# bdsaglam/torch-scae

Hardware: AMD Instinct MI355X
Metric: images/sec SCAE fwd+bwd, MNIST 40x40 bs=128, 1/2/4/8 MI355X (higher is better)
Workload: dtype f32

## Files before the change

include/scae_hip.h:

```cpp
#ifndef SCAE_HIP_H
#define SCAE_HIP_H

#include <stdint.h>

#ifdef __cplusplus
extern "C" {
#endif

#define SCAE_ABI_VERSION 3

#define SCAE_OK 0
#define SCAE_ERR_BAD_ARG (-1)
#define SCAE_ERR_UNSUPPORTED (-2)

#define SCAE_MAX_CHANNELS 4
#define SCAE_ATTN_MAX_SET 64
#define SCAE_RENDER_MAX_TEMPLATE_ELEMS 4096

int scae_abi_version(void);
const char *scae_error_string(int code);

void *scae_launch_list_begin(void *stream);
int scae_launch_list_end(void *list);
int scae_launch_list_size(const void *list);
// ... 188 lines not shown
  const float *all_param;
  const float *cpr_static, *bias_cvr, *bias_caps, *bias_vote, *bias_scale;
  const float *noise_caps, *noise_vote;
  float noise_scale;
  int V, ld_param, similarity, learn_vote_scale, allow_deformations;
  float *vote, *scale, *vote_presence, *logit_caps, *logit_vote, *reg_partial;
  float *caps_presence;
  int *caps_arg;
  const float *gvote, *gscale, *gvote_presence, *glogit_caps, *glogit_vote, *greg;
  const float *gcaps_presence;
  float *gall_param, *gcpr_in, *gall_param_gated;
} scae_votes_desc;
int scae_mlp_chain_votes_fwd_f32(const scae_mlp_chain_desc *desc, const scae_votes_desc *votes,
                                 void *stream);
int scae_mlp_chain_votes_bwd_f32(const scae_mlp_chain_desc *desc, const scae_votes_desc *votes,
                                 void *stream);

int scae_gemm_bf16(const float *A, const float *B, float *C, const float *bias,
                   const float *mask, float *asum, int batch, int M, int N, int K,
                   int a_kcontig, int lda, int64_t a_batch, int b_kcontig, int ldb,
                   int64_t b_batch, int ldc, int64_t c_batch, int bias_ld, int64_t bias_batch,
                   int ldmask, int64_t mask_batch, int64_t asum_batch, int asum_ld, int relu,
                   void *stream);
int scae_gemm_pair_bf16(const scae_gemm_desc *first, const scae_gemm_desc *second, void *stream);
int scae_gemm_multi_bf16(const scae_gemm_desc *descs, int n, void *stream);
int scae_conv3x3_fwd_fold_f32(const float *in, const float *wf, const float *bias, float *out,
                              const float *post_bias, float *out_post, int B, int IH, int IW,
                              int Cin, int Cout, int stride, const scae_seed_fold_desc *fold,
                              void *stream);
int scae_conv3x3_fwd_res_supported(int B, int IH, int IW, int Cin, int Cout, int stride);
int scae_conv3x3_fwd_res_f32(const float *in, const float *wp, const float *bias, float *out,
                             const float *post_bias, float *out_post, int B, int IH, int IW,
                             int Cin, int Cout, int stride, int group, void *stream);
int scae_conv3x3_fwd_bf16(const float *in, const float *wf, const float *bias, float *out,
                          const float *post_bias, float *out_post, int B, int IH, int IW, int Cin,
                          int Cout, int stride, void *stream);
int scae_conv3x3_bwd_pair_bf16(const float *dpre, const float *wd, const float *in, float *din,
                               float *partial, int B, int IH, int IW, int Cin, int Cout,
                               int stride, void *stream);

int64_t scae_conv3x3_wf_floats(int Cout, int Cin);
int scae_conv3x3_relayout_f32(const float *w, float *wf, float *wd, int Cout, int Cin,
                              void *stream);

int scae_conv3x3_bf16r_supported(int B, int IH, int IW, int Cin, int Cout, int stride);
int scae_conv3x3_first_fwd_relayout_bf16(const float *img, const float *w, const float *bias,
                                         uint16_t *out_h, int B, int Cin, int IH, int IW,
                                         int Cout, int stride, int n_layers,
                                         const float *const *rw, float *const *rwf,
                                         float *const *rwd, uint16_t *const *rwfh,
                                         uint16_t *const *rwdh, const int *rCout,
                                         const int *rCin, void *stream);
int scae_cvt_bf16_batch(int n_arrays, const float *const *src, uint16_t *const *dst,
                        const int64_t *n, void *stream);
int scae_conv3x3_fwd_bf16r(const uint16_t *in, const uint16_t *wf, const float *bias,
                           uint16_t *out_h, float *out_f, const float *post_bias,
                           float *out_post, int B, int IH, int IW, int Cin, int Cout, int stride,
                           void *stream);
int scae_conv3x3_dgrad_bf16r(const uint16_t *dpre, const uint16_t *wd, const uint16_t *gate,
                             uint16_t *din_h, float *din_f, int B, int IH, int IW, int Cin,
                             int Cout, int stride, void *stream);
int scae_conv3x3_wgrad_bf16r_splits(int B, int OH, int OW, int Cin, int Cout);
int scae_conv3x3_wgrad_bf16r(const uint16_t *dpre, const uint16_t *x, float *partial, int B,
                             int IH, int IW, int Cin, int Cout, int stride, void *stream);
int scae_conv3x3_relayout_batch_f32(int n_layers, const float *const *w, float *const *wf,
                                    float *const *wd, const int *Cout, const int *Cin,
// ... 555 lines not shown
```

torch_scae_amd/_lib.py:

```python
import ctypes
import os
from ctypes import (POINTER, Structure, c_char_p, c_double, c_float, c_int,
                    c_int64, c_uint32, c_uint64, c_void_p)

_HERE = os.path.dirname(os.path.abspath(__file__))
LIB_PATH = os.environ.get("SCAE_HIP_LIB") or os.path.join(_HERE, "lib",
                                                        "libscae_hip.so")

P = c_void_p


class DecoderDesc(Structure):
    _fields_ = [("templates", P), ("templates_alpha", P), ("pose", P),
                ("presence", P), ("bg_image", P), ("bg_value", P),
                ("bg_mixing_logit", P), ("temperature_logit", P),
                ("out_scale", P),
                ("B", c_int), ("M", c_int), ("C", c_int), ("th", c_int),
                ("tw", c_int), ("H", c_int), ("W", c_int),
                ("template_repeat", c_int)]


class LikelihoodBwdDesc(Structure):
    _fields_ = [(n, P) for n in (
        "vote", "scale", "vote_presence", "dummy_vote", "x", "presence",
# ... 174 lines not shown
    "scae_gemm_pair_f32": [POINTER(GemmDesc), POINTER(GemmDesc), P],
    "scae_launch_list_begin": [P],
    "scae_launch_list_end": [P],
    "scae_launch_list_size": [P],
    "scae_launch_list_run": [P, P],
    "scae_launch_list_lane": [P, c_int],
    "scae_launch_list_timeline": [P, P, P, POINTER(c_float), c_int],
    "scae_launch_list_free": [P],
    "scae_gemm_multi_f32": [POINTER(GemmDesc), c_int, P],
    "scae_gemm_multi_bf16": [POINTER(GemmDesc), c_int, P],
    "scae_mlp_chain_max_width": [],
    "scae_mlp_chain_fwd_f32": [POINTER(MlpChainDesc), P],
    "scae_mlp_chain_bwd_f32": [POINTER(MlpChainDesc), P],
    "scae_mlp_chain_votes_fwd_f32": [POINTER(MlpChainDesc), POINTER(VotesDesc), P],
    "scae_mlp_chain_votes_bwd_f32": [POINTER(MlpChainDesc), POINTER(VotesDesc), P],
    "scae_gemm_pair_bf16": [POINTER(GemmDesc), POINTER(GemmDesc), P],
    "scae_conv3x3_wf_floats": [c_int, c_int],
    "scae_conv3x3_relayout_f32": [P, P, P, c_int, c_int, P],
    "scae_conv3x3_bf16r_supported": [c_int] * 6,
    "scae_conv3x3_first_fwd_relayout_bf16": [P] * 4 + [c_int] * 7 + [P] * 8,
    "scae_cvt_bf16_batch": [c_int, P, P, P, P],
    "scae_conv3x3_fwd_bf16r": [P] * 7 + [c_int] * 6 + [P],
    "scae_conv3x3_dgrad_bf16r": [P] * 5 + [c_int] * 6 + [P],
    "scae_conv3x3_wgrad_bf16r_splits": [c_int] * 5,
    "scae_conv3x3_wgrad_bf16r": [P] * 3 + [c_int] * 6 + [P],
    "scae_conv3x3_relayout_batch_f32": [c_int, P, P, P, P, P, P],
    "scae_conv3x3_first_fwd_f32": [P] * 4 + [c_int] * 6 + [P],
    "scae_conv3x3_first_fwd_relayout_f32": [P] * 4 + [c_int] * 7 + [P] * 6,
    "scae_conv3x3_first_wgrad_reduce_f32": [P] * 3 + [c_int] * 7 + [P] * 7,
    "scae_conv3x3_first_wgrad_rows": [c_int] * 2,
    "scae_conv3x3_first_wgrad_f32": [P] * 3 + [c_int] * 6 + [P],
    "scae_conv3x3_fwd_f32": [P] * 6 + [c_int] * 6 + [P],
    "scae_conv3x3_fwd_fold_f32": [P] * 6 + [c_int] * 6 + [POINTER(SeedFoldDesc), P],
    "scae_conv3x3_fwd_res_supported": [c_int] * 6,
    "scae_conv3x3_fwd_res_f32": [P] * 6 + [c_int] * 7 + [P],
    "scae_conv3x3_fwd_bf16": [P] * 6 + [c_int] * 6 + [P],
    "scae_conv3x3_dgrad_f32": [P] * 4 + [c_int] * 6 + [P],
    "scae_conv3x3_bwd_pair_f32": [P] * 5 + [c_int] * 6 + [P],
    "scae_conv3x3_bwd_pair_reduce_f32": [P] * 5 + [c_int] * 6 + [P, c_int] + [P] * 7
    + [c_int] * 2 + [P],
    "scae_conv3x3_bwd_pair_fold_f32": [P] * 5 + [c_int] * 6
    + [POINTER(SeedFoldDesc), POINTER(SeedFoldGrads), P],
    "scae_conv3x3_bwd_pair_bf16": [P] * 5 + [c_int] * 6 + [P],
    "scae_conv3x3_wgrad_reduce_batch_f32": [c_int] + [P] * 7,
    "scae_conv3x3_wgrad_splits": [c_int] * 5,
    "scae_conv3x3_wgrad_f32": [P] * 5 + [c_int] * 6 + [P],
    "scae_attention_pool_supported": [c_int] * 3,
    "scae_attention_pool_fwd_f32": [P, P] + [c_int] * 4 + [P],
    "scae_attention_pool_bwd_f32": [P, P, P] + [c_int] * 4 + [P],
    "scae_stage_batch": [P, P, c_int64, P, P, c_int64, P],
    "scae_step_prologue_f32": [P, P, c_int64, P, P, c_int64, P, c_int64, P,
                               POINTER(SeedFoldDesc), P],
    "scae_step_prologue_first_f32": [P, P, c_int64, P, P, c_int64, P, c_int64,
                                     P, POINTER(SeedFoldDesc),
                                     POINTER(FirstLayerDesc), P],
    "scae_gather_batch_f32": [P, P, c_int, POINTER(BatchSourceDesc), P],
    "scae_step_prologue_source_f32": [P, P, c_int, POINTER(BatchSourceDesc), P, c_int64, P,
                                      POINTER(SeedFoldDesc), POINTER(FirstLayerDesc), P],
    "scae_rmsprop_step_f32": [P, P, P, P, c_int64, c_float, P, c_float, c_float,
                              c_float, c_float, c_float, P],
    "scae_rmsprop_sums_step_f32": [P, P, P, P, c_int64, c_float, P, c_float, c_float,
                                   c_float, c_float, POINTER(SumJob), c_int, P],
    "scae_flat_opt_step_f32": [P, P, P, P, P, c_int64, P, P, c_int, c_double, c_double, c_float,
                               c_float, c_float, c_int, c_float, c_int, P],
    "scae_flat_opt_sums_step_f32": [P, P, P, P, P, c_int64, P, P, c_int, c_double, c_double,
                                    c_float, c_float, c_int, c_float, POINTER(SumJob), c_int, P],
# ... 204 lines not shown
```

torch_scae_amd/csrc/conv_mfma.hip:

```cpp
#include <cstdlib>

#include "mfma_tile.h"
#include "mfma_pipe.h"
#include "conv_first_dev.h"
#include "seed_fold_dev.h"

#include <algorithm>

#include "wave_mfma.h"

#define SCAE_DEVICE_ONLY
namespace scae_sf {
#include "seed_fold.hip"
}
namespace scae_saw {
#include "seed_attention_wave.hip"
}
#undef SCAE_DEVICE_ONLY

namespace {
using namespace scae_tile;

using scae_first::ConvGeom;

// ... 801 lines not shown
      for (int j = 0; j < 4; ++j)
        pipe::dma16(ra, reinterpret_cast<float *>(stage + 8 * j * ROWB), va[j], sa);
    } else {
#pragma unroll
      for (int j = 0; j < 4; ++j) {
        const int row = 8 * j + (lane >> 3);
        const int dh = pih[j] - kh, dw = piw[j] - kw, oh = dh >> 1, ow = dw >> 1;
        const bool ok = pn[j] >= 0 && dh >= 0 && dw >= 0 && oh < g.OH && ow < g.OW;
        const int vv = ok ? ((pn[j] + oh * g.OW + ow) * g.Cout) * 4 + swz(row, lane & 7) * 16
                          : pipe::DMA_ZERO;
        pipe::dma16(ra, reinterpret_cast<float *>(stage + 8 * j * ROWB), vv, h * BKF * 4);
      }
    }
#pragma unroll
    for (int j = 0; j < 8; ++j)
      pipe::dma16(rb, reinterpret_cast<float *>(stage + A_B + 8 * j * ROWB), vb[j], sb);
  });
  const int row = tid >> 3, c8 = 8 * (tid & 7), m = m0 + row;
  if (m >= M) return;
  const int nb = m / (AH * AW), rem = m - nb * AH * AW, a = rem / AW, b = rem - a * AW;
  const int ih = pl.rlist[pl.rstart[rc] + a], iw = pl.clist[pl.cstart[cc] + b];
  const size_t o = (((size_t)nb * g.IH + ih) * g.IW + iw) * g.Cin + n0 + c8;
  if (gate) {
    const float4 g0 = ld4(gate + o), g1 = ld4(gate + o + 4);
    v.lo.x = g0.x > 0.f ? v.lo.x : 0.f, v.lo.y = g0.y > 0.f ? v.lo.y : 0.f;
    v.lo.z = g0.z > 0.f ? v.lo.z : 0.f, v.lo.w = g0.w > 0.f ? v.lo.w : 0.f;
    v.hi.x = g1.x > 0.f ? v.hi.x : 0.f, v.hi.y = g1.y > 0.f ? v.hi.y : 0.f;
    v.hi.z = g1.z > 0.f ? v.hi.z : 0.f, v.hi.w = g1.w > 0.f ? v.hi.w : 0.f;
  }
  *reinterpret_cast<float4 *>(din + o) = v.lo;
  *reinterpret_cast<float4 *>(din + o + 4) = v.hi;
}

template <int DMODE>
struct DgradShape {
  static constexpr int SMEM = Tile<DMODE>::SMEM;
};
template <>
struct DgradShape<4> {
  static constexpr int SMEM = dgx::SMEM;
};
template <>
struct DgradShape<5> {
  static constexpr int SMEM = dgk::SMEM;
};
template <int DMODE, int SM>
__device__ __forceinline__ void dgrad_any_tile(float *smem, int bx, int by,
                                               const float *__restrict__ dpre,
                                               const float *__restrict__ wd,
                                               const float *__restrict__ gate,
                                               float *__restrict__ din, const ConvGeom &g,
                                               const DgradPlan &pl) {
  if constexpr (DMODE == 4)
    dgrad_x6_tile<(SM >= 2 * dgx::SMEM ? 2 : 1)>(smem, bx, by, dpre, wd, gate, din, g, pl);
  else if constexpr (DMODE == 5)
    dgrad_x6k_tile(smem, bx, by, dpre, wd, gate, din, g, pl);
  else
    dgrad_tile<DMODE>(smem, bx, by, dpre, wd, gate, din, g, pl);
}

template <int NS>
__global__ __launch_bounds__(NT) void conv_dgrad_x6_kernel(const float *__restrict__ dpre,
                                                           const float *__restrict__ wd,
                                                           const float *__restrict__ gate,
                                                           float *__restrict__ din, ConvGeom g,
                                                           DgradPlan pl) {
// ... 399 lines not shown
  if (lds > 64 * 1024) return SCAE_ERR_UNSUPPORTED;
  ReduceBatch r{};
  int rb = 0;
  if (n_layers > 0) {
    rb = fill_reduce(r, n_layers, rpartial, rdw, rdb, rCout, rCin, rsplits);
    SCAE_REQUIRE(rb > 0);
  }
  const int n_first = B * f.slices;
#define SCAE_FIRST_WGRAD(CI)                                                                  \
  case CI:                                                                                    \
    scae::launch(conv_first_wgrad_kernel<CI>, dim3(n_first + n_layers * rb), dim3(256), \
                       lds, (hipStream_t)stream, dpre, img, partial, g, r, n_first, rb);      \
    break;
  switch (Cin) {
    SCAE_FIRST_WGRAD(1) SCAE_FIRST_WGRAD(2) SCAE_FIRST_WGRAD(3) SCAE_FIRST_WGRAD(4)
    default: return SCAE_ERR_UNSUPPORTED;
  }
#undef SCAE_FIRST_WGRAD
  return scae_launch_status();
}

extern "C" int scae_conv3x3_first_wgrad_f32(const float *dpre, const float *img, float *partial,
                                            int B, int Cin, int IH, int IW, int Cout, int stride,
                                            void *stream) {
  return scae_conv3x3_first_wgrad_reduce_f32(dpre, img, partial, B, Cin, IH, IW, Cout, stride, 0,
                                             nullptr, nullptr, nullptr, nullptr, nullptr, nullptr,
                                             stream);
}

static bool conv_bf16_shape(long rows, int Cin, int Cout) {
  return Cin % 128 == 0 && Cout % 128 == 0 && rows * (Cout / 128) >= 128 * 128;
}

static int conv_fwd_impl(const float *in, const float *wf, const float *bias, float *out,
                         const float *post_bias, float *out_post, int B, int IH, int IW, int Cin,
                         int Cout, int stride, bool bf16, void *stream) {
  ConvGeom g{B, IH, IW, (IH - 3) / stride + 1, (IW - 3) / stride + 1, Cin, Cout, stride};
  int rc = check_geom(g, true);
  if (rc) return rc;
  SCAE_REQUIRE(in && wf && bias && out && (!out_post || post_bias));
  const int M = B * g.OH * g.OW;
  hipStream_t st = (hipStream_t)stream;
  if (bf16 && conv_bf16_shape(M, Cin, Cout)) {
    scae::launch(conv_fwd_kernel<3>, dim3(Cout / 128, (M + 127) / 128), dim3(NT), 0, st, in,
                       wf, bias, out, post_bias, out_post, g);
    return scae_launch_status();
  }
  scae::launch(conv_fwd_pipe_kernel<PipeC2>, dim3(Cout / PipeC2::TB, (M + PipeC2::TA - 1) / PipeC2::TA),
               dim3(pipe::NT), 0, st, in, wf, bias, out, post_bias, out_post, g);
  return scae_launch_status();
}

extern "C" int scae_conv3x3_fwd_f32(const float *in, const float *wf, const float *bias,
                                    float *out, const float *post_bias, float *out_post, int B,
                                    int IH, int IW, int Cin, int Cout, int stride,
                                    void *stream) {
  return conv_fwd_impl(in, wf, bias, out, post_bias, out_post, B, IH, IW, Cin, Cout, stride,
                       false, stream);
}
extern "C" int scae_conv3x3_fwd_fold_f32(const float *in, const float *wf, const float *bias,
                                         float *out, const float *post_bias, float *out_post,
                                         int B, int IH, int IW, int Cin, int Cout, int stride,
                                         const scae_seed_fold_desc *fold, void *stream) {
  SCAE_REQUIRE(in && wf && bias && out && fold && B > 0 && stride > 0 && IH >= 3 && IW >= 3);
  if (Cin % pipe::BK || Cout % PipeC2::TB) return SCAE_ERR_UNSUPPORTED;
  const scae_seed_fold_desc &a = *fold;
  if (!(a.seeds && a.wq && a.bq && a.wk && a.bk && a.wv && a.bv && a.wo && a.bo && a.w2 && a.b2 &&
        a.q && a.wkf && a.bkf && a.wvf && a.bvf && a.wv2e))
    return SCAE_ERR_BAD_ARG;
  if (!scae_seed_fold_supported(a.O, a.C, a.D) ||
      scae_fold::lds_bytes(a.C, a.D) > FOLD_SMEM * sizeof(float))
    return SCAE_ERR_UNSUPPORTED;
  ConvGeom g{B, IH, IW, (IH - 3) / stride + 1, (IW - 3) / stride + 1, Cin, Cout, stride};
  const scae_fold::Plan plan = scae_fold::plan(a.C, a.D);
  const int M = B * g.OH * g.OW, gx = Cout / PipeC2::TB,
            n_conv = gx * ((M + PipeC2::TA - 1) / PipeC2::TA);
  scae::launch(conv_fwd_pipe_fold_kernel<PipeC2>, dim3(n_conv + plan.blocks()),
                     dim3(pipe::NT), 0, (hipStream_t)stream, in, wf, bias, out, post_bias, out_post,
                     g, gx, n_conv, a, plan);
  return scae_launch_status();
}

extern "C" int scae_conv3x3_fwd_bf16(const float *in, const float *wf, const float *bias,
                                     float *out, const float *post_bias, float *out_post, int B,
                                     int IH, int IW, int Cin, int Cout, int stride,
                                     void *stream) {
  return conv_fwd_impl(in, wf, bias, out, post_bias, out_post, B, IH, IW, Cin, Cout, stride,
                       true, stream);
}

struct DgradLaunch {
  DgradPlan pl;
  int mode, gx, ny;
};
#ifndef SCAE_DGK_DEFAULT
#define SCAE_DGK_DEFAULT 1
#endif
#ifndef SCAE_DGX_MIN_TILES
#define SCAE_DGX_MIN_TILES 500
#endif
#ifndef SCAE_PAIR_SMALL_TILES
#define SCAE_PAIR_SMALL_TILES SCAE_SMALL_TILES
#endif
#ifndef SCAE_PAIR_WIDE_MIN
#define SCAE_PAIR_WIDE_MIN 600
#endif
static DgradLaunch plan_dgrad(const ConvGeom &g, bool pair = false, bool bf16 = false) {
// ... 205 lines not shown
```

torch_scae_amd/csrc/conv_resident.hip:

```cpp
#include <cstdlib>

#include "bf16x6.h"
#include "mfma_pipe.h"
#include "conv_first_dev.h"

namespace {
namespace pipe = scae_pipe;
using scae_first::ConvGeom;
constexpr int NT = 256;

struct ResArgs {
  const float *in, *wp, *bias, *post_bias;
  float *out, *out_post;
  ConvGeom g;
  int G;
};

template <int MI>
__global__ __launch_bounds__(NT, 2) void conv_res_fwd_kernel(ResArgs a) {
  constexpr bool X6 = true;
  extern __shared__ __attribute__((aligned(1024))) float smem[];
  const int tid = threadIdx.x, wid = __builtin_amdgcn_readfirstlane(tid >> 6), lane = tid & 63,
            li = lane & 31, lk = lane >> 5;
  const ConvGeom &g = a.g;
  const int ntiles = g.Cout / 32;
  const int nt = blockIdx.x % ntiles, img0 = (blockIdx.x / ntiles) * a.G;
  const int nimg = min(a.G, g.B - img0);
  const int ipix = g.IH * g.IW, opix = g.OH * g.OW;
  const int SP = g.Cin / 4;
  {
    const pipe::rsrc_t rin =
        pipe::make_rsrc(a.in, (unsigned)((size_t)g.B * ipix * g.Cin * 4));
    const int units = a.G * ipix * SP, pieces = (units + 63) / 64;
    const int valid = nimg * ipix;
    for (int j = wid; j < pieces; j += 4) {
      const int u = j * 64 + lane, p = u / SP, s = u - p * SP;
      const int vo = p < valid ? (((img0 * ipix + p) * g.Cin) + ((s ^ (p & 15)) << 2)) * 4
                               : pipe::DMA_ZERO;
      pipe::dma16(rin, smem + j * 256, vo, 0);
    }
  }
  const int rows = nimg * opix;
  int pbase[MI];
#pragma unroll
  for (int mi = 0; mi < MI; ++mi) {
    const int r = min(mi * 32 + li, rows - 1);
    const int n = r / opix, rem = r - n * opix, oh = rem / g.OW, ow = rem - oh * g.OW;
    pbase[mi] = n * ipix + oh * g.stride * g.IW + ow * g.stride;
  }
  const int CB = g.Cin / 32;
  const int CPT = CB / 4;
  const int NCW = 9 * CPT;
  const uint4 *wq = reinterpret_cast<const uint4 *>(a.wp) + (size_t)nt * (9 * CB) * 384 + lane;
  constexpr int NS = !X6 ? 1 : (MI == 1 ? 3 : 1);
  pipe::f32x16 acc[MI], accl[X6 ? MI : 1][NS];
#pragma unroll
  for (int mi = 0; mi < MI; ++mi)
#pragma unroll
    for (int e = 0; e < 16; ++e) {
// ... 76 lines not shown
#pragma unroll
    for (int e = 0; e < 16; ++e) smem[((wid * MI + mi) * 16 + e) * 64 + lane] = acc[mi][e];
  const int col = nt * 32 + li;
  const float bn = a.bias[col];
  float pb[MI][4];
  const int row0 = 8 * wid + 4 * lk;
  if (a.out_post) {
#pragma unroll
    for (int mi = 0; mi < MI; ++mi)
#pragma unroll
      for (int e = 0; e < 4; ++e) {
        const int r = min(mi * 32 + row0 + e, rows - 1);
        pb[mi][e] = a.post_bias[(size_t)col * opix + r % opix];
      }
  }
  __syncthreads();
  const unsigned obytes = (unsigned)((size_t)g.B * opix * g.Cout * 4);
  const pipe::rsrc_t ro = pipe::make_rsrc(a.out, obytes);
  const pipe::rsrc_t rp = pipe::make_rsrc(a.out_post ? a.out_post : a.out, obytes);
#pragma unroll
  for (int mi = 0; mi < MI; ++mi)
#pragma unroll
    for (int e = 0; e < 4; ++e) {
      float v = 0.f;
#pragma unroll
      for (int w = 0; w < 4; ++w) v += smem[((w * MI + mi) * 16 + 4 * wid + e) * 64 + lane];
      const int r = mi * 32 + row0 + e;
      const float o = fmaxf(v + bn, 0.f);
      const int off = r < rows ? ((img0 * opix + r) * g.Cout + col) * 4 : pipe::DMA_ZERO;
      __builtin_amdgcn_raw_buffer_store_b32(__builtin_bit_cast(int, o), ro, off, 0, 0);
      if (a.out_post)
        __builtin_amdgcn_raw_buffer_store_b32(__builtin_bit_cast(int, o + pb[mi][e]), rp, off, 0, 0);
    }
}

struct ResPlan {
  int G, MI;
  size_t lds;
};
bool res_plan(const ConvGeom &g, ResPlan &p, int force_g) {
  if (g.stride < 1 || g.stride > 2 || g.Cin % 128 || g.Cout % 32) return false;
  const int opix = g.OH * g.OW, ipix = g.IH * g.IW;
  double best = 0.;
  p.G = 0;
  for (int G = 1; G <= 8 && G <= g.B; ++G) {
    if (force_g > 0 && G != force_g) continue;
    const int MI = (G * opix + 31) / 32;
    const size_t stage = ((size_t)G * ipix * g.Cin * 4 + 1023) & ~(size_t)1023;
    const size_t lds = std::max(stage, (size_t)4 * MI * 16 * 64 * 4);
    if (MI > 4 || lds > (force_g > 0 ? 150 : 64) * 1024) break;
    const double use = (double)G * opix / (32. * MI);
    if (use > best + 1e-9) best = use, p.G = G, p.MI = MI, p.lds = lds;
  }
  return p.G > 0;
}
}

extern "C" int scae_conv3x3_fwd_res_supported(int B, int IH, int IW, int Cin, int Cout, int stride) {
  if (B <= 0 || IH < 3 || IW < 3 || Cin <= 0 || Cout <= 0 || stride <= 0) return 0;
  ConvGeom g{B, IH, IW, (IH - 3) / stride + 1, (IW - 3) / stride + 1, Cin, Cout, stride};
  ResPlan p;
  return res_plan(g, p, 0) ? 1 : 0;
}

extern "C" int scae_conv3x3_fwd_res_f32(const float *in, const float *wp, const float *bias,
                                        float *out, const float *post_bias, float *out_post, int B,
                                        int IH, int IW, int Cin, int Cout, int stride, int group,
                                        void *stream) {
  SCAE_REQUIRE(in && wp && bias && out && (!out_post || post_bias) && B > 0 && IH >= 3 && IW >= 3 &&
               Cin > 0 && Cout > 0 && stride > 0 && group >= 0);
  ConvGeom g{B, IH, IW, (IH - 3) / stride + 1, (IW - 3) / stride + 1, Cin, Cout, stride};
  ResPlan p;
  if (!res_plan(g, p, group)) return SCAE_ERR_UNSUPPORTED;
  ResArgs a{in, wp, bias, post_bias, out, out_post, g, p.G};
  const dim3 grid((Cout / 32) * ((B + p.G - 1) / p.G));
  hipStream_t st = (hipStream_t)stream;
#define SCAE_RES(M)                                                                              \
  case M: {                                                                                      \
    if (p.lds > 48 * 1024) {                                                                     \
      hipError_t e = hipFuncSetAttribute(reinterpret_cast<const void *>(conv_res_fwd_kernel<M>), \
                                         hipFuncAttributeMaxDynamicSharedMemorySize, (int)p.lds); \
      if (e != hipSuccess) return (int)e;                                                        \
    }                                                                                            \
    scae::launch(conv_res_fwd_kernel<M>, grid, dim3(NT), p.lds, st, a);                          \
    break;                                                                                       \
  }
  switch (p.MI) {
    SCAE_RES(1) SCAE_RES(2) SCAE_RES(3) SCAE_RES(4)
    default: return SCAE_ERR_UNSUPPORTED;
  }
#undef SCAE_RES
  return scae_launch_status();
}
```

torch_scae_amd/ops.py:

```python
import ctypes
import functools

import numpy as np
import torch

from . import _lib, step_plan
from ._lib import DecoderDesc, ScaeHipError
from .step_plan import StepPlan, current as _plan

__all__ = ["geometric_transform", "qkv_attention", "set_encoder", "grouped_mlp", "seed_attention", "seed_attention_supported", "seed_fold", "seed_fold_supported", "loss_tail", "loss_tail_scalar", "loss_tail_supported", "capsule_votes",
           "capsule_likelihood", "colored_templates", "template_color_supported", "attention_conv_pool", "attention_pool_supported", "capsule_head", "part_encoder", "conv_stack", "conv_stack_supported",
           "uniform", "reset_noise", "pack_params", "render_templates", "render_gmm_log_prob", "render_gmm_log_prob_sums",
           "gmm_log_prob", "gmm_mean", "gmm_mode", "render_gmm_mode", "image_sheet", "ScaeHipError"]


def _need_hip(*tensors):
    for t in tensors:
        if t is None:
            continue
        if not t.is_cuda:
            raise ScaeHipError(
                "torch_scae_amd ops run only on a HIP device (got a "
                f"{t.device} tensor); there is no CPU path.")
        if t.dtype != torch.float32:
# ... 53 lines not shown
    return torch.empty(shape, device=like.device, dtype=like.dtype)


def _in_slot(t):
    return t is not None and getattr(t, "_scae_in_slot", False)


def _sum_jobs(jobs):
    arr = (_lib.ScaledSum * max(1, len(jobs)))()
    for a, (src, scale, dst) in zip(arr, jobs):
        assert src.is_contiguous() and dst.numel() == 1
        a.src, a.n, a.scale, a.dst = src.data_ptr(), src.numel(), scale, \
            dst.data_ptr()
    return arr


def scaled_sums(jobs):
    _lib.call("scae_scaled_sums_f32", _sum_jobs(jobs), len(jobs),
              _stream(jobs[0][0]))


def mfma_bf16(enabled=True):
    return _plan().precision(enabled)


def _bf16():
    return _plan().bf16


def _prec(name):
    return name.replace("_f32", "_bf16") if _plan().bf16 else name


_FOLD_RIDES = __import__("os").environ.get("SCAE_FOLD_RIDES", "conv")


class StepPrologue:

    def __init__(self):
        self.noise = self.noise_state = None
        self.fold_inputs = self.fold_outs = self.fold_dims = None
        self.first_inputs = self.first_outs = None
        self.first_half = None
        self.noise_fresh = self.fold_fresh = self.first_fresh = False
        self.fold_rides_conv = False
        self.fold_conv_ok = False if _FOLD_RIDES == "prologue" else None

    def _first_desc(self, image):
        _, weights, biases, strides = self.first_inputs
        act, wfs, wds = self.first_outs
        d = _lib.FirstLayerDesc()
        d.img, d.w, d.bias, d.out = image.data_ptr(), weights[0].data_ptr(), \
            biases[0].data_ptr(), act.data_ptr()
        d.B, d.Cin, d.IH, d.IW = image.shape
        d.Cout, d.stride, d.n_layers = weights[0].shape[0], strides[0], len(wfs)
        for i, (w, wf, wd) in enumerate(zip(weights[1:], wfs, wds)):
            d.rw[i], d.rwf[i], d.rwd[i] = w.data_ptr(), wf.data_ptr(), \
                wd.data_ptr()
            d.rCout[i], d.rCin[i] = w.shape[0], w.shape[1]
        if self.first_half is not None:
            act_h, wfh, wdh = self.first_half
            d.out_h = act_h.data_ptr()
            for i, (a, b) in enumerate(zip(wfh, wdh)):
                d.rwfh[i], d.rwdh[i] = a.data_ptr(), b.data_ptr()
        return d

    def launch(self, dst_image=None, src_image=None, dst_label=None,
               src_label=None, stream_ref=None, source=None):
        stage = dst_image is not None
        n_noise = 0 if self.noise is None else self.noise.numel()
        first = self.first_outs is not None and (
            not stage or (dst_image.data_ptr() == self.first_inputs[0].data_ptr()
                          and dst_image.shape == self.first_inputs[0].shape))
        if not (stage or n_noise or self.fold_outs is not None or first):
            return
        ref = dst_image if stage else (
            self.noise if n_noise else (self.fold_outs[0] if self.fold_outs
                                        is not None else self.first_outs[0]))
        _need_hip(ref)
# ... 744 lines not shown
            halves = (half(B, oh, ow, c1),
                      [half(w.shape[0], 9, w.shape[1]) for w in weights[1:]],
                      [half(w.shape[1], 9, w.shape[0]) for w in weights[1:]])
        if pro is not None:
            pro.first_inputs = (image, list(weights), list(biases),
                                tuple(strides))
            pro.first_outs = (act, wfs, wds)
            pro.first_half = halves
    if pro is not None:
        pro.first_fresh = False
    acts = [act]
    n = L - 1
    if launch:
        arr = lambda ts: (ctypes.c_void_p * max(n, 1))(
            *[t.data_ptr() for t in ts])
        ints = lambda v: (ctypes.c_int * max(n, 1))(*v)
        if resident:
            _lib.call("scae_conv3x3_first_fwd_relayout_bf16", _p(image),
                      _p(weights[0]), _p(biases[0]), _p(halves[0]), B, C0, H, W,
                      c1, s, n, arr(weights[1:]), arr(wfs), arr(wds),
                      arr(halves[1]), arr(halves[2]),
                      ints([w.shape[0] for w in weights[1:]]),
                      ints([w.shape[1] for w in weights[1:]]), st)
        else:
            _lib.call("scae_conv3x3_first_fwd_relayout_f32", _p(image),
                      _p(weights[0]), _p(biases[0]), _p(act), B, C0, H, W, c1, s,
                      n, arr(weights[1:]), arr(wfs), arr(wds),
                      ints([w.shape[0] for w in weights[1:]]),
                      ints([w.shape[1] for w in weights[1:]]), st)
    x_post = None
    if resident:
        return _conv_stack_fwd_bf16r(halves, weights, biases, strides,
                                     post_bias, image.dtype)
    for l in range(1, L):
        w, s = weights[l], strides[l]
        co, ci = w.shape[0], w.shape[1]
        ih, iw = act.shape[1], act.shape[2]
        out = new(B, (ih - 3) // s + 1, (iw - 3) // s + 1, co)
        if l == L - 1 and post_bias is not None:
            x_post = torch.empty_like(out)
        conv = (_p(act), _p(wfs[l - 1]), _p(biases[l]), _p(out),
                _p(post_bias if x_post is not None else None), _p(x_post), B,
                ih, iw, ci, co, s)
        carried = False
        if l == 1 and pro is not None and pro.fold_outs is not None:
            if _bf16() or pro.fold_conv_ok is False:
                pro.fold_rides_conv = False
            elif pro.fold_fresh:
                pro.fold_rides_conv = True
            else:
                rc = _lib.load().scae_conv3x3_fwd_fold_f32(
                    *conv, ctypes.byref(_fold_desc(
                        pro.fold_inputs, pro.fold_outs, *pro.fold_dims)), st)
                if rc == _lib.ERR_UNSUPPORTED:
                    pro.fold_conv_ok = pro.fold_rides_conv = False
                else:
                    _lib.check(rc, "scae_conv3x3_fwd_fold_f32")
                    carried = pro.fold_fresh = pro.fold_rides_conv = True
        if not carried:
            if not _bf16() and _conv_resident(B, ih, iw, ci, co, s):
                _lib.call("scae_conv3x3_fwd_res_f32", _p(act),
                          _p(wfs[l - 1][1]), *conv[2:], 0, st)
            else:
                _lib.call(_prec("scae_conv3x3_fwd_f32"), *conv, st)
        acts.append(out)
        act = out
    return acts, wds, x_post


_CONV_BF16R = __import__("os").environ.get("SCAE_CONV_BF16R", "1") != "0"



def _conv_bf16_resident(B, ih, iw, weights, strides):
    if not (_bf16() and _CONV_BF16R and len(strides) >= 2):
        return False
    lib = _lib.load()
    for l in range(1, len(strides)):
        co, ci, s = weights[l].shape[0], weights[l].shape[1], strides[l]
        if not lib.scae_conv3x3_bf16r_supported(B, ih, iw, ci, co, s):
            return False
        ih, iw = (ih - 3) // s + 1, (iw - 3) // s + 1
    return True


def _cvt_bf16(pairs, ref):
    for k in range(0, len(pairs), 8):
        chunk = pairs[k:k + 8]
        n = len(chunk)
        _lib.call("scae_cvt_bf16_batch", n,
                  (ctypes.c_void_p * n)(*[a.data_ptr() for a, _ in chunk]),
                  (ctypes.c_void_p * n)(*[b.data_ptr() for _, b in chunk]),
                  (ctypes.c_int64 * n)(*[a.numel() for a, _ in chunk]),
                  _stream(ref))


def _conv_stack_fwd_bf16r(halves, weights, biases, strides, post_bias, dt):
# ... 2103 lines not shown
```

Before: 265,100.

## Ride seed-fold blocks on resident conv and add K-split forward conv kernel

Lets the seed-attention fold work share a grid with the resident conv forward kernel, hosted on the last layer that qualifies for the resident path rather than always on layer 1 through the pipe kernel. This removes a separate launch and lets fold blocks overlap conv blocks. Separately, adds an x6 K-split forward conv kernel, with a fold variant, which becomes the default non-resident f32 path whenever the channel counts divide the tile sizes. The combined grid raises LDS and occupancy pressure, and the fold now depends on some layer passing the resident check.

```diff
diff --git a/include/scae_hip.h b/include/scae_hip.h
--- a/include/scae_hip.h
+++ b/include/scae_hip.h
@@ -244,6 +244,14 @@
 int scae_conv3x3_fwd_res_f32(const float *in, const float *wp, const float *bias, float *out,
                              const float *post_bias, float *out_post, int B, int IH, int IW,
                              int Cin, int Cout, int stride, int group, void *stream);
+int scae_conv3x3_fwd_res_fold_f32(const float *in, const float *wp, const float *bias, float *out,
+                                  const float *post_bias, float *out_post, int B, int IH, int IW,
+                                  int Cin, int Cout, int stride, int group,
+                                  const scae_seed_fold_desc *fold, void *stream);
+int scae_conv3x3_fwd_ksplit_takes(int B, int IH, int IW, int Cin, int Cout, int stride);
+int scae_conv3x3_fwd_ksplit_f32(const float *in, const float *wf, const float *bias, float *out,
+                                const float *post_bias, float *out_post, int B, int IH, int IW,
+                                int Cin, int Cout, int stride, void *stream);
 int scae_conv3x3_fwd_bf16(const float *in, const float *wf, const float *bias, float *out,
                           const float *post_bias, float *out_post, int B, int IH, int IW, int Cin,
                           int Cout, int stride, void *stream);
diff --git a/torch_scae_amd/_lib.py b/torch_scae_amd/_lib.py
--- a/torch_scae_amd/_lib.py
+++ b/torch_scae_amd/_lib.py
@@ -230,6 +230,9 @@
     "scae_conv3x3_first_wgrad_f32": [P] * 3 + [c_int] * 6 + [P],
     "scae_conv3x3_fwd_f32": [P] * 6 + [c_int] * 6 + [P],
     "scae_conv3x3_fwd_fold_f32": [P] * 6 + [c_int] * 6 + [POINTER(SeedFoldDesc), P],
+    "scae_conv3x3_fwd_ksplit_takes": [c_int] * 6,
+    "scae_conv3x3_fwd_ksplit_f32": [P] * 6 + [c_int] * 6 + [P],
+    "scae_conv3x3_fwd_res_fold_f32": [P] * 6 + [c_int] * 7 + [POINTER(SeedFoldDesc), P],
     "scae_conv3x3_fwd_res_supported": [c_int] * 6,
     "scae_conv3x3_fwd_res_f32": [P] * 6 + [c_int] * 7 + [P],
     "scae_conv3x3_fwd_bf16": [P] * 6 + [c_int] * 6 + [P],
diff --git a/torch_scae_amd/csrc/conv_mfma.hip b/torch_scae_amd/csrc/conv_mfma.hip
--- a/torch_scae_amd/csrc/conv_mfma.hip
+++ b/torch_scae_amd/csrc/conv_mfma.hip
@@ -857,6 +857,92 @@
   *reinterpret_cast<float4 *>(din + o + 4) = v.hi;
 }
 
+__device__ __forceinline__ void fwd_x6k_tile(float *smemf, int bx, int by,
+                                             const float *__restrict__ in,
+                                             const float *__restrict__ wf,
+                                             const float *__restrict__ bias,
+                                             float *__restrict__ out,
+                                             const float *__restrict__ post_bias,
+                                             float *__restrict__ out_post, const ConvGeom &g) {
+  using namespace dgk;
+  using dgx::swz;
+  const int tid = threadIdx.x, lane = tid & 63;
+  const int M = g.B * g.OH * g.OW, hw = g.OH * g.OW;
+  const int m0 = by * TM, n0 = bx * TN;
+  const pipe::rsrc_t ra = pipe::make_rsrc(in, (unsigned)((size_t)g.B * g.IH * g.IW * g.Cin * 4));
+  const pipe::rsrc_t rb = pipe::make_rsrc(wf, (unsigned)((size_t)g.Cout * 9 * g.Cin * 4));
+  int va[4], vb[8];
+#pragma unroll
+  for (int j = 0; j < 4; ++j) {
+    const int row = 8 * j + (lane >> 3), m = m0 + row;
+    va[j] = pipe::DMA_ZERO;
+    if (m < M) {
+      const int n = m / hw, rem = m - n * hw, oh = rem / g.OW, ow = rem - oh * g.OW;
+      va[j] = (((n * g.IH + oh * g.stride) * g.IW + ow * g.stride) * g.Cin) * 4 +
+              swz(row, lane & 7) * 16;
+    }
+  }
+#pragma unroll
+  for (int j = 0; j < 8; ++j) {
+    const int row = 8 * j + (lane >> 3);
+    vb[j] = ((n0 + row) * 9 * g.Cin) * 4 + swz(row, lane & 7) * 16;
+  }
+  const int cpt = g.Cin / BKF;
+  const Out8 v = pipeline(smemf, 9 * cpt, [&](int c, unsigned char *stage) {
+    const int tap = c / cpt, h = c - tap * cpt, kh = tap / 3, kw = tap - kh * 3;
+    const int sa = ((kh * g.IW + kw) * g.Cin + h * BKF) * 4, sb = (tap * g.Cin + h * BKF) * 4;
+#pragma unroll
+    for (int j = 0; j < 4; ++j)
+      pipe::dma16(ra, reinterpret_cast<float *>(stage + 8 * j * ROWB), va[j], sa);
+#pragma unroll
+    for (int j = 0; j < 8; ++j)
+      pipe::dma16(rb, reinterpret_cast<float *>(stage + A_B + 8 * j * ROWB), vb[j], sb);
+  });
+  const int row = tid >> 3, c8 = 8 * (tid & 7), m = m0 + row, n = n0 + c8;
+  const float4 b0 = ld4(bias + n), b1 = ld4(bias + n + 4);
+  float pb[8];
+  if (out_post) {
+    const float *src = post_bias + (size_t)n * hw + min(m, M - 1) % hw;
+#pragma unroll
+    for (int e = 0; e < 8; ++e) pb[e] = src[(size_t)e * hw];
+  }
+  const float o[8] = {fmaxf(v.lo.x + b0.x, 0.f), fmaxf(v.lo.y + b0.y, 0.f), fmaxf(v.lo.z + b0.z, 0.f),
+                      fmaxf(v.lo.w + b0.w, 0.f), fmaxf(v.hi.x + b1.x, 0.f), fmaxf(v.hi.y + b1.y, 0.f),
+                      fmaxf(v.hi.z + b1.z, 0.f), fmaxf(v.hi.w + b1.w, 0.f)};
+  const unsigned obytes = (unsigned)((size_t)M * g.Cout * 4);
+  const pipe::rsrc_t ro = pipe::make_rsrc(out, obytes);
+  const pipe::rsrc_t rp = pipe::make_rsrc(out_post ? out_post : out, obytes);
+  const int off = (m * g.Cout + n) * 4;
+#pragma unroll
+  for (int e = 0; e < 8; ++e)
+    __builtin_amdgcn_raw_buffer_store_b32(__builtin_bit_cast(int, o[e]), ro, off + 4 * e, 0, 0);
+  if (out_post) {
+#pragma unroll
+    for (int e = 0; e < 8; ++e)
+      __builtin_amdgcn_raw_buffer_store_b32(__builtin_bit_cast(int, o[e] + pb[e]), rp, off + 4 * e,
+                                            0, 0);
+  }
+}
+__global__ __launch_bounds__(NT) void conv_fwd_x6k_kernel(
+    const float *__restrict__ in, const float *__restrict__ wf, const float *__restrict__ bias,
+    float *__restrict__ out, const float *__restrict__ post_bias, float *__restrict__ out_post,
+    ConvGeom g) {
+  __shared__ __attribute__((aligned(1024))) float smem[dgk::SMEM];
+  fwd_x6k_tile(smem, blockIdx.x, blockIdx.y, in, wf, bias, out, post_bias, out_post, g);
+}
+__global__ __launch_bounds__(NT, 3) void conv_fwd_x6k_fold_kernel(
+    const float *__restrict__ in, const float *__restrict__ wf, const float *__restrict__ bias,
+    float *__restrict__ out, const float *__restrict__ post_bias, float *__restrict__ out_post,
+    ConvGeom g, int gx, int n_conv, scae_seed_fold_desc fold, scae_fold::Plan plan) {
+  static_assert(dgk::SMEM >= FOLD_SMEM, "the riders' LDS");
+  __shared__ __attribute__((aligned(1024))) float smem[dgk::SMEM];
+  const int blk = blockIdx.x;
+  if (blk < n_conv)
+    fwd_x6k_tile(smem, blk % gx, blk / gx, in, wf, bias, out, post_bias, out_post, g);
+  else
+    scae_fold::forward_block_any<16>(fold, plan, blk - n_conv, smem);
+}
+
 template <int DMODE>
 struct DgradShape {
   static constexpr int SMEM = Tile<DMODE>::SMEM;
@@ -1322,9 +1408,16 @@
   return Cin % 128 == 0 && Cout % 128 == 0 && rows * (Cout / 128) >= 128 * 128;
 }
 
+static bool fwd_ksplit(const ConvGeom &g) {
+  return g.Cin % dgk::BKF == 0 && g.Cout % dgk::TN == 0 &&
+         (size_t)g.B * g.IH * g.IW * g.Cin * 4 < (1u << 31) &&
+         (size_t)g.B * g.OH * g.OW * g.Cout * 4 < (1u << 31);
+}
+
 static int conv_fwd_impl(const float *in, const float *wf, const float *bias, float *out,
                          const float *post_bias, float *out_post, int B, int IH, int IW, int Cin,
-                         int Cout, int stride, bool bf16, void *stream) {
+                         int Cout, int stride, bool bf16, void *stream,
+                         bool force_ksplit = false) {
   ConvGeom g{B, IH, IW, (IH - 3) / stride + 1, (IW - 3) / stride + 1, Cin, Cout, stride};
   int rc = check_geom(g, true);
   if (rc) return rc;
@@ -1336,9 +1429,28 @@
                        wf, bias, out, post_bias, out_post, g);
     return scae_launch_status();
   }
+  if (force_ksplit && !fwd_ksplit(g)) return SCAE_ERR_UNSUPPORTED;
+  if (fwd_ksplit(g)) {
+    scae::launch(conv_fwd_x6k_kernel, dim3(Cout / dgk::TN, (M + dgk::TM - 1) / dgk::TM), dim3(NT),
+                 0, st, in, wf, bias, out, post_bias, out_post, g);
+    return scae_launch_status();
+  }
   scae::launch(conv_fwd_pipe_kernel<PipeC2>, dim3(Cout / PipeC2::TB, (M + PipeC2::TA - 1) / PipeC2::TA),
                dim3(pipe::NT), 0, st, in, wf, bias, out, post_bias, out_post, g);
   return scae_launch_status();
+}
+
+extern "C" int scae_conv3x3_fwd_ksplit_takes(int B, int IH, int IW, int Cin, int Cout, int stride) {
+  if (B <= 0 || IH < 3 || IW < 3 || Cin <= 0 || Cout <= 0 || stride <= 0) return 0;
+  ConvGeom g{B, IH, IW, (IH - 3) / stride + 1, (IW - 3) / stride + 1, Cin, Cout, stride};
+  return check_geom(g, true) == SCAE_OK && fwd_ksplit(g) ? 1 : 0;
+}
+extern "C" int scae_conv3x3_fwd_ksplit_f32(const float *in, const float *wf, const float *bias,
+                                           float *out, const float *post_bias, float *out_post,
+                                           int B, int IH, int IW, int Cin, int Cout, int stride,
+                                           void *stream) {
+  return conv_fwd_impl(in, wf, bias, out, post_bias, out_post, B, IH, IW, Cin, Cout, stride,
+                       false, stream, true);
 }
 
 extern "C" int scae_conv3x3_fwd_f32(const float *in, const float *wf, const float *bias,
@@ -1363,6 +1475,12 @@
     return SCAE_ERR_UNSUPPORTED;
   ConvGeom g{B, IH, IW, (IH - 3) / stride + 1, (IW - 3) / stride + 1, Cin, Cout, stride};
   const scae_fold::Plan plan = scae_fold::plan(a.C, a.D);
+  if (fwd_ksplit(g)) {
+    const int M = B * g.OH * g.OW, gx = Cout / dgk::TN, n_conv = gx * ((M + dgk::TM - 1) / dgk::TM);
+    scae::launch(conv_fwd_x6k_fold_kernel, dim3(n_conv + plan.blocks()), dim3(NT), 0,
+                 (hipStream_t)stream, in, wf, bias, out, post_bias, out_post, g, gx, n_conv, a, plan);
+    return scae_launch_status();
+  }
   const int M = B * g.OH * g.OW, gx = Cout / PipeC2::TB,
             n_conv = gx * ((M + PipeC2::TA - 1) / PipeC2::TA);
   scae::launch(conv_fwd_pipe_fold_kernel<PipeC2>, dim3(n_conv + plan.blocks()),
diff --git a/torch_scae_amd/csrc/conv_resident.hip b/torch_scae_amd/csrc/conv_resident.hip
--- a/torch_scae_amd/csrc/conv_resident.hip
+++ b/torch_scae_amd/csrc/conv_resident.hip
@@ -3,6 +3,7 @@
 #include "bf16x6.h"
 #include "mfma_pipe.h"
 #include "conv_first_dev.h"
+#include "seed_fold_dev.h"
 
 namespace {
 namespace pipe = scae_pipe;
@@ -17,14 +18,13 @@
 };
 
 template <int MI>
-__global__ __launch_bounds__(NT, 2) void conv_res_fwd_kernel(ResArgs a) {
+__device__ __forceinline__ void res_fwd_block(const ResArgs &a, float *smem, int blk) {
   constexpr bool X6 = true;
-  extern __shared__ __attribute__((aligned(1024))) float smem[];
   const int tid = threadIdx.x, wid = __builtin_amdgcn_readfirstlane(tid >> 6), lane = tid & 63,
             li = lane & 31, lk = lane >> 5;
   const ConvGeom &g = a.g;
   const int ntiles = g.Cout / 32;
-  const int nt = blockIdx.x % ntiles, img0 = (blockIdx.x / ntiles) * a.G;
+  const int nt = blk % ntiles, img0 = (blk / ntiles) * a.G;
   const int nimg = min(a.G, g.B - img0);
   const int ipix = g.IH * g.IW, opix = g.OH * g.OW;
   const int SP = g.Cin / 4;
@@ -167,6 +167,24 @@
       if (a.out_post)
         __builtin_amdgcn_raw_buffer_store_b32(__builtin_bit_cast(int, o + pb[mi][e]), rp, off, 0, 0);
     }
+}
+
+template <int MI>
+__global__ __launch_bounds__(NT, 2) void conv_res_fwd_kernel(ResArgs a) {
+  extern __shared__ __attribute__((aligned(1024))) float smem[];
+  res_fwd_block<MI>(a, smem, blockIdx.x);
+}
+
+template <int MI>
+__global__ __launch_bounds__(NT, MI <= 2 ? 3 : 2) void conv_res_fwd_fold_kernel(ResArgs a, int n_fold,
+                                                                  scae_seed_fold_desc fold,
+                                                                  scae_fold::Plan plan) {
+  extern __shared__ __attribute__((aligned(1024))) float smem[];
+  const int blk = blockIdx.x;
+  if (blk < n_fold)
+    scae_fold::forward_block_any<16>(fold, plan, blk, smem);
+  else
+    res_fwd_block<MI>(a, smem, blk - n_fold);
 }
 
 struct ResPlan {
@@ -198,26 +216,48 @@
   return res_plan(g, p, 0) ? 1 : 0;
 }
 
-extern "C" int scae_conv3x3_fwd_res_f32(const float *in, const float *wp, const float *bias,
-                                        float *out, const float *post_bias, float *out_post, int B,
-                                        int IH, int IW, int Cin, int Cout, int stride, int group,
-                                        void *stream) {
+static int conv_res_launch(const float *in, const float *wp, const float *bias, float *out,
+                           const float *post_bias, float *out_post, int B, int IH, int IW, int Cin,
+                           int Cout, int stride, int group, const scae_seed_fold_desc *fold,
+                           void *stream) {
   SCAE_REQUIRE(in && wp && bias && out && (!out_post || post_bias) && B > 0 && IH >= 3 && IW >= 3 &&
                Cin > 0 && Cout > 0 && stride > 0 && group >= 0);
   ConvGeom g{B, IH, IW, (IH - 3) / stride + 1, (IW - 3) / stride + 1, Cin, Cout, stride};
   ResPlan p;
   if (!res_plan(g, p, group)) return SCAE_ERR_UNSUPPORTED;
+  scae_fold::Plan fp{};
+  int n_fold = 0;
+  if (fold) {
+    const scae_seed_fold_desc &f = *fold;
+    if (!(f.seeds && f.wq && f.bq && f.wk && f.bk && f.wv && f.bv && f.wo && f.bo && f.w2 && f.b2 &&
+          f.q && f.wkf && f.bkf && f.wvf && f.bvf && f.wv2e))
+      return SCAE_ERR_BAD_ARG;
+    if (!scae_seed_fold_supported(f.O, f.C, f.D)) return SCAE_ERR_UNSUPPORTED;
+    const size_t fl = (scae_fold::lds_bytes(f.C, f.D) + 1023) & ~(size_t)1023;
+    if (fl > p.lds && (p.MI > 2 || 3 * fl > 160 * 1024)) return SCAE_ERR_UNSUPPORTED;
+    p.lds = std::max(p.lds, fl);
+    fp = scae_fold::plan(f.C, f.D);
+    n_fold = fp.blocks();
+  }
   ResArgs a{in, wp, bias, post_bias, out, out_post, g, p.G};
-  const dim3 grid((Cout / 32) * ((B + p.G - 1) / p.G));
+  const int n_conv = (Cout / 32) * ((B + p.G - 1) / p.G);
   hipStream_t st = (hipStream_t)stream;
+#define SCAE_RES_LDS(K)                                                                          \
+  if (p.lds > 48 * 1024) {                                                                       \
+    hipError_t e = hipFuncSetAttribute(reinterpret_cast<const void *>(K),                        \
+                                       hipFuncAttributeMaxDynamicSharedMemorySize, (int)p.lds);  \
+    if (e != hipSuccess) return (int)e;                                                          \
+  }
 #define SCAE_RES(M)                                                                              \
   case M: {                                                                                      \
-    if (p.lds > 48 * 1024) {                                                                     \
-      hipError_t e = hipFuncSetAttribute(reinterpret_cast<const void *>(conv_res_fwd_kernel<M>), \
-                                         hipFuncAttributeMaxDynamicSharedMemorySize, (int)p.lds); \
-      if (e != hipSuccess) return (int)e;                                                        \
+    if (fold) {                                                                                  \
+      SCAE_RES_LDS(conv_res_fwd_fold_kernel<M>)                                                  \
+      scae::launch(conv_res_fwd_fold_kernel<M>, dim3(n_fold + n_conv), dim3(NT), p.lds, st, a,   \
+                   n_fold, *fold, fp);                                                           \
+    } else {                                                                                     \
+      SCAE_RES_LDS(conv_res_fwd_kernel<M>)                                                       \
+      scae::launch(conv_res_fwd_kernel<M>, dim3(n_conv), dim3(NT), p.lds, st, a);                \
     }                                                                                            \
-    scae::launch(conv_res_fwd_kernel<M>, grid, dim3(NT), p.lds, st, a);                          \
     break;                                                                                       \
   }
   switch (p.MI) {
@@ -225,5 +265,23 @@
     default: return SCAE_ERR_UNSUPPORTED;
   }
 #undef SCAE_RES
+#undef SCAE_RES_LDS
   return scae_launch_status();
 }
+
+extern "C" int scae_conv3x3_fwd_res_f32(const float *in, const float *wp, const float *bias,
+                                        float *out, const float *post_bias, float *out_post, int B,
+                                        int IH, int IW, int Cin, int Cout, int stride, int group,
+                                        void *stream) {
+  return conv_res_launch(in, wp, bias, out, post_bias, out_post, B, IH, IW, Cin, Cout, stride,
+                         group, nullptr, stream);
+}
+extern "C" int scae_conv3x3_fwd_res_fold_f32(const float *in, const float *wp, const float *bias,
+                                             float *out, const float *post_bias, float *out_post,
+                                             int B, int IH, int IW, int Cin, int Cout, int stride,
+                                             int group, const scae_seed_fold_desc *fold,
+                                             void *stream) {
+  SCAE_REQUIRE(fold);
+  return conv_res_launch(in, wp, bias, out, post_bias, out_post, B, IH, IW, Cin, Cout, stride,
+                         group, fold, stream);
+}
diff --git a/torch_scae_amd/ops.py b/torch_scae_amd/ops.py
--- a/torch_scae_amd/ops.py
+++ b/torch_scae_amd/ops.py
@@ -109,9 +109,6 @@
     return name.replace("_f32", "_bf16") if _plan().bf16 else name
 
 
-_FOLD_RIDES = __import__("os").environ.get("SCAE_FOLD_RIDES", "conv")
-
-
 class StepPrologue:
 
     def __init__(self):
@@ -121,7 +118,7 @@
         self.first_half = None
         self.noise_fresh = self.fold_fresh = self.first_fresh = False
         self.fold_rides_conv = False
-        self.fold_conv_ok = False if _FOLD_RIDES == "prologue" else None
+        self.fold_conv_ok = None
 
     def _first_desc(self, image):
         _, weights, biases, strides = self.first_inputs
@@ -932,6 +929,19 @@
     if resident:
         return _conv_stack_fwd_bf16r(halves, weights, biases, strides,
                                      post_bias, image.dtype)
+    fold_host = None
+    if pro is not None and pro.fold_outs is not None:
+        if _bf16() or pro.fold_conv_ok is False:
+            pro.fold_rides_conv = False
+        else:
+            ih, iw = act.shape[1], act.shape[2]
+            for l in range(1, L):
+                co, ci, s = weights[l].shape[0], weights[l].shape[1], strides[l]
+                if _conv_resident(B, ih, iw, ci, co, s):
+                    fold_host = l
+                ih, iw = (ih - 3) // s + 1, (iw - 3) // s + 1
+            if fold_host is None:
+                pro.fold_conv_ok = pro.fold_rides_conv = False
     for l in range(1, L):
         w, s = weights[l], strides[l]
         co, ci = w.shape[0], w.shape[1]
@@ -942,27 +952,25 @@
         conv = (_p(act), _p(wfs[l - 1]), _p(biases[l]), _p(out),
                 _p(post_bias if x_post is not None else None), _p(x_post), B,
                 ih, iw, ci, co, s)
-        carried = False
-        if l == 1 and pro is not None and pro.fold_outs is not None:
-            if _bf16() or pro.fold_conv_ok is False:
-                pro.fold_rides_conv = False
-            elif pro.fold_fresh:
-                pro.fold_rides_conv = True
-            else:
-                rc = _lib.load().scae_conv3x3_fwd_fold_f32(
-                    *conv, ctypes.byref(_fold_desc(
-                        pro.fold_inputs, pro.fold_outs, *pro.fold_dims)), st)
-                if rc == _lib.ERR_UNSUPPORTED:
-                    pro.fold_conv_ok = pro.fold_rides_conv = False
+        if not _bf16() and _conv_resident(B, ih, iw, ci, co, s):
+            res = (_p(act), _p(wfs[l - 1][1]), *conv[2:], 0)
+            carried = False
+            if l == fold_host:
+                if pro.fold_fresh:
+                    pro.fold_rides_conv = True
                 else:
-                    _lib.check(rc, "scae_conv3x3_fwd_fold_f32")
-                    carried = pro.fold_fresh = pro.fold_rides_conv = True
-        if not carried:
-            if not _bf16() and _conv_resident(B, ih, iw, ci, co, s):
-                _lib.call("scae_conv3x3_fwd_res_f32", _p(act),
-                          _p(wfs[l - 1][1]), *conv[2:], 0, st)
-            else:
-                _lib.call(_prec("scae_conv3x3_fwd_f32"), *conv, st)
+                    rc = _lib.load().scae_conv3x3_fwd_res_fold_f32(
+                        *res, ctypes.byref(_fold_desc(
+                            pro.fold_inputs, pro.fold_outs, *pro.fold_dims)), st)
+                    if rc == _lib.ERR_UNSUPPORTED:
+                        pro.fold_conv_ok = pro.fold_rides_conv = False
+                    else:
+                        _lib.check(rc, "scae_conv3x3_fwd_res_fold_f32")
+                        carried = pro.fold_fresh = pro.fold_rides_conv = True
+            if not carried:
+                _lib.call("scae_conv3x3_fwd_res_f32", *res, st)
+        else:
+            _lib.call(_prec("scae_conv3x3_fwd_f32"), *conv, st)
         acts.append(out)
         act = out
     return acts, wds, x_post
```

Result: no change. 265,100, median of 2 (+0.0%).
